# tenpy/cyten

Hardware: AMD Instinct MI355X
Metric: block-sparse tdot+SVD GFLOP/s (fp64) (higher is better)
Workload: dtype f64

## Files before the change

### cyten_amd/csrc/jacobi_engine.hip

```cpp
#include "jacobi_engine.h"

#include <algorithm>
#include <cmath>
#include <cstdlib>

namespace cyb {
constexpr double kPredictQuad = 16.0;
namespace {

typedef double d4 __attribute__((ext_vector_type(4)));
typedef double d2 __attribute__((ext_vector_type(2)));
#define GLOBAL_AS __attribute__((address_space(1)))
typedef const GLOBAL_AS d2* gc2;
typedef const GLOBAL_AS d2* gcp2;
typedef GLOBAL_AS double* gp;

constexpr int GS = JP + 2;
constexpr int QS = JP + 16;
constexpr int GK = 64;
constexpr int XS = GK + 2;
constexpr int NT = 256;
constexpr int NPAIR = JP / 2;
static_assert(JP == 32, "the wave tiling below assumes 32 x 32 pair problems");

// ... 818 lines not shown
                if (ab > 1e-300) {
                    jacobi_rot_bf(Hr[p * CS + p], Hr[q * CS + q], ab, c, sn, thr2);
                    pr = gr / ab;
                    pi = gi / ab;
                }
                rot[lane * 4 + 0] = c;
                rot[lane * 4 + 1] = sn;
                rot[lane * 4 + 2] = pr;
                rot[lane * 4 + 3] = pi;
            }
            __builtin_amdgcn_fence(__ATOMIC_RELEASE, "wavefront");
            __builtin_amdgcn_wave_barrier();
            for (int e = lane; e < (CJ / 2) * CJ; e += 64) {
                const int k = e / CJ, col = e % CJ;
                int p, q;
                pair_of(r, k, p, q);
                const double c = rot[k * 4], sn = rot[k * 4 + 1], fr = rot[k * 4 + 2], fi = rot[k * 4 + 3];
                const double pr_ = Hr[p * CS + col], pi_ = Hi[p * CS + col], qr_ = Hr[q * CS + col], qi_ = Hi[q * CS + col];
                const double tr = fr * qr_ - fi * qi_, ti = fr * qi_ + fi * qr_;
                Hr[p * CS + col] = c * pr_ - sn * tr;
                Hi[p * CS + col] = c * pi_ - sn * ti;
                Hr[q * CS + col] = sn * pr_ + c * tr;
                Hi[q * CS + col] = sn * pi_ + c * ti;
            }
            __builtin_amdgcn_fence(__ATOMIC_RELEASE, "wavefront");
            __builtin_amdgcn_wave_barrier();
            for (int e = lane; e < (CJ / 2) * CJ * 2; e += 64) {
                const int which = e / ((CJ / 2) * CJ), f = e % ((CJ / 2) * CJ);
                const int k = f / CJ, row = f % CJ;
                int p, q;
                pair_of(r, k, p, q);
                double* Xr = which ? Ur : Hr;
                double* Xi = which ? Ui : Hi;
                const double c = rot[k * 4], sn = rot[k * 4 + 1], fr = rot[k * 4 + 2], fi = -rot[k * 4 + 3];
                const double pr_ = Xr[row * CS + p], pi_ = Xi[row * CS + p], qr_ = Xr[row * CS + q], qi_ = Xi[row * CS + q];
                const double tr = fr * qr_ - fi * qi_, ti = fr * qi_ + fi * qr_;
                Xr[row * CS + p] = c * pr_ - sn * tr;
                Xi[row * CS + p] = c * pi_ - sn * ti;
                Xr[row * CS + q] = sn * pr_ + c * tr;
                Xi[row * CS + q] = sn * pi_ + c * ti;
            }
            __builtin_amdgcn_fence(__ATOMIC_RELEASE, "wavefront");
            __builtin_amdgcn_wave_barrier();
        }
    for (int e = lane; e < CJ * CJ; e += 64) {
        const int a = e / CJ, b = e % CJ;
        const double x = Ur[a * CS + b], y = Ui[a * CS + b];
        Vout[(2 * a) * VS + 2 * b] = x;
        Vout[(2 * a) * VS + 2 * b + 1] = -y;
        Vout[(2 * a + 1) * VS + 2 * b] = y;
        Vout[(2 * a + 1) * VS + 2 * b + 1] = x;
    }
    if (lane < CJ) {
        const double lam = Hr[lane * CS + lane];
        Gdiag[(2 * lane) * GS + 2 * lane] = lam;
        Gdiag[(2 * lane + 1) * GS + 2 * lane + 1] = lam;
    }
}

struct SScratch {
    double* gpart;
    unsigned int* ticket;
    unsigned int* ready;
    unsigned int* err;
    const int2* wgmap;
    const int2* wgent;
    unsigned long long* stamps;
    int stamp_round;
    int n_sweeps, n_mats;
    unsigned int* arrive;
    int* nsw;
    unsigned int* readyJ;
    int defer_j;
    int cross_every, cross_min_nb;
};
constexpr int SW_MAX_ENT = 64;

constexpr int SW_UN = 8;
constexpr int SW_PRE = 6;
constexpr int SWEEP_XREG = (4 * JP * GS > JP * GS + 2 * JP * VS) ? 4 * JP * GS : JP * GS + 2 * JP * VS;
constexpr int SWEEP_LDS_DOUBLES = JP * GS + SWEEP_XREG + 2 * JP * QS + 8;
constexpr size_t SWEEP_LDS_BYTES = 88 * 1024;
static_assert((size_t)SWEEP_LDS_DOUBLES * 8 + 1024 <= SWEEP_LDS_BYTES, "LDS request of the sweep kernel");
constexpr int SWEEP_WG_PER_CU = 1;

typedef unsigned int u32x2 __attribute__((ext_vector_type(2)));
union Q8 {
    u32x2 u;
    double d;
};

template <int SLEEP = 1>
__device__ __forceinline__ bool spin_until(const unsigned int* word, unsigned int target, unsigned int* err)
{
    const unsigned long long t0 = wall_clock64();
    unsigned int it = 0;
    while (__hip_atomic_load(word, __ATOMIC_RELAXED, __HIP_MEMORY_SCOPE_AGENT) < target) {
        __builtin_amdgcn_s_sleep(SLEEP);
        if ((++it & 63u) == 0u) {
            if (__hip_atomic_load(err, __ATOMIC_RELAXED, __HIP_MEMORY_SCOPE_AGENT) != 0u) return false;
            if (wall_clock64() - t0 > 100000000ull) {
                __hip_atomic_store(err, 1u, __ATOMIC_RELAXED, __HIP_MEMORY_SCOPE_AGENT);
                return false;
            }
        }
    }
    return true;
}

__device__ __forceinline__ void sweep_update_j(const __amdgpu_buffer_rsrc_t rsJ, const double* Qm, int P, int Q, int nvp, int j_begin,
                                               int nJ, int wave, int lane)
{
    const int un = lane & 15, ukq = lane >> 4;
    const double* ap0 = Qm + (lane >> 4) * QS + (lane & 15);
    const double* ap1 = ap0 + 16;
    double a0[JP / 4], a1[JP / 4];
#pragma unroll
    for (int kk = 0; kk < JP / 4; ++kk) {
        a0[kk] = ap0[kk * 4 * QS];
        a1[kk] = ap1[kk * 4 * QS];
    }
    auto off_of = [&](int c, int k) { return (unsigned int)(((int64_t)xrow(k, P, Q) * nvp + (j_begin + c) * 64 + wave * 16 + un) * 8); };
    auto load = [&](double (&x)[JP / 4], int c) {
#pragma unroll
        for (int kk = 0; kk < JP / 4; ++kk) {
            Q8 q;
            q.u = __builtin_amdgcn_raw_buffer_load_b64(rsJ, off_of(c, 4 * kk + ukq), 0, 16);
            x[kk] = q.d;
        }
    };
    double xb[JP / 4], xn[JP / 4];
    if (nJ > 0) load(xb, 0);
    for (int c = 0; c < nJ; ++c) {
        if (c + 1 < nJ) load(xn, c + 1);
        d4 acc[2] = {d4{0.0, 0.0, 0.0, 0.0}, d4{0.0, 0.0, 0.0, 0.0}};
#pragma unroll
        for (int kk = 0; kk < JP / 4; ++kk) {
            acc[0] = __builtin_amdgcn_mfma_f64_16x16x4f64(a0[kk], xb[kk], acc[0], 0, 0, 0);
            acc[1] = __builtin_amdgcn_mfma_f64_16x16x4f64(a1[kk], xb[kk], acc[1], 0, 0, 0);
        }
#pragma unroll
        for (int i = 0; i < 2; ++i)
#pragma unroll
            for (int q = 0; q < 4; ++q) {
                Q8 v;
                v.d = acc[i][q];
                __builtin_amdgcn_raw_buffer_store_b64(v.u, rsJ, off_of(c, i * 16 + (lane >> 4) + 4 * q), 0, 16);
            }
#pragma unroll
        for (int kk = 0; kk < JP / 4; ++kk) xb[kk] = xn[kk];
    }
}

template <bool CPLX>
__global__ void __launch_bounds__(NT, 1)
jacobi_sweep_kernel(const RPair* __restrict__ pairs, int max_inner, unsigned long long* __restrict__ offmax_bits, SScratch sc)
{
    extern __shared__ __attribute__((aligned(16))) double rsm[];
    double* Gs = rsm;
    double* G2 = Gs + JP * GS;
    double* Va = G2 + JP * GS;
    double* Vb = Va + JP * VS;
    double* Xc = G2;
    double* Qs0 = G2 + SWEEP_XREG;
    double* Qs1 = Qs0 + JP * QS;
    double* red = Qs1 + JP * QS;
    int* ibase = reinterpret_cast<int*>(red + 8);
    int* perm = ibase;
    int* zrow = ibase + JP;
    int* zout = ibase + 2 * JP;
    int* flags = ibase + 3 * JP;
    int* edone = flags + 4;

    const int tid = threadIdx.x;
    const int lane = tid & 63, wave = tid >> 6;
    const int2 went = sc.wgent ? sc.wgent[blockIdx.x] : make_int2((int)blockIdx.x, (int)blockIdx.x + 1);
    int max_rounds = 0;
    for (int e = went.x; e < went.y; ++e) max_rounds = max(max_rounds, pairs[sc.wgmap[e].x].nb - 1);
    const int n_sw = sc.n_sweeps;
    const bool one_entry = went.y - went.x == 1;
    int pendP = -1, pendQ = -1, pend_ground = 0;
    if (n_sw > 1) {
        if (tid < SW_MAX_ENT) edone[tid] = 0;
        __syncthreads();
    }
    for (int sw = 0; sw < n_sw; ++sw) {
    for (int round = 0; round < max_rounds; ++round)
    for (int ent = went.x; ent < went.y; ++ent) {
    const int2 wm = sc.wgmap[ent];
    const int pi = wm.x, part = wm.y;
    const RPair mt = pairs[pi];
    if (round >= mt.nb - 1) continue;
    if (n_sw > 1 && edone[ent - went.x]) continue;
    const int ground = sw * (mt.nb - 1) + round;
    const int G = mt.pad[0];
    unsigned int* ready = sc.ready + mt.pad[1];
    unsigned int* readyJ = sc.readyJ + mt.pad[1];
    unsigned int* ticket = sc.ticket + pi;
    double* Qs = (ground & 1) ? Qs1 : Qs0;
    const unsigned int pbytes = JP * JP * 8;
    const __amdgpu_buffer_rsrc_t rsW = __builtin_amdgcn_make_buffer_rsrc(mt.W, 0, (int)((size_t)mt.nvp * mt.lenp * 8), 0x00020000);
    const __amdgpu_buffer_rsrc_t rsJ =
        __builtin_amdgcn_make_buffer_rsrc(mt.J ? mt.J : mt.W, 0, mt.J ? (int)((size_t)mt.nvp * mt.nvp * 8) : 0, 0x00020000);
    const int cw = mt.lenp / 64, cj = mt.J ? mt.nvp / 64 : 0;
    const int w_begin = (int)((int64_t)part * cw / G), w_end = (int)((int64_t)(part + 1) * cw / G);
    const int j_begin = (int)((int64_t)part * cj / G), j_end = (int)((int64_t)(part + 1) * cj / G);
    const int nW = w_end - w_begin, nJ = j_end - j_begin;
    const bool defer = sc.defer_j && one_entry && G > 1 && nJ > 0 && round < mt.nb - 2;
    const int ct = defer ? nW : nW + nJ;
    const int pre_limit = (sc.defer_j && G > 1) ? min(ct, nW) : ct;
    const int un = lane & 15, ukq = lane >> 4;
#define SWEEP_STAMP(k)                                                                                            \
    do {                                                                                                          \
        if (sc.stamps && tid == 0 && round == sc.stamp_round) sc.stamps[(size_t)blockIdx.x * 8 + (k)] = wall_clock64(); \
    } while (0)

    {
        int P, Q;
        circle_pair(mt.nb, round, mt.slot, P, Q);
        if (P > Q) {
            const int t = P;
            P = Q;
            Q = t;
        }
        SWEEP_STAMP(0);
        __syncthreads();
        if (ground > 0) {
            if (tid == 0) {
                bool ok = spin_until(ready + (size_t)P * G + part, (unsigned int)ground, sc.err);
                ok = ok && spin_until(ready + (size_t)Q * G + part, (unsigned int)ground, sc.err);
                flags[1] = ok ? 1 : 0;
            }
            __syncthreads();
            if (!flags[1]) return;
        }
        SWEEP_STAMP(1);
        auto chunk_off = [&](int c, int k, bool& in_w) -> unsigned int {
            in_w = c < nW;
            const int ld = in_w ? mt.lenp : mt.nvp;
            const int cc = in_w ? w_begin + c : j_begin + (c - nW);
            return (unsigned int)(((int64_t)xrow(k, P, Q) * ld + cc * 64 + wave * 16 + un) * 8);
        };
        auto chunk_load = [&](int c, int k) -> double {
            bool in_w;
            const unsigned int off = chunk_off(c, k, in_w);
            Q8 q;
            q.u = in_w ? __builtin_amdgcn_raw_buffer_load_b64(rsW, off, 0, 16) : __builtin_amdgcn_raw_buffer_load_b64(rsJ, off, 0, 16);
            return q.d;
        };
        double xpre[SW_PRE][JP / 4];
        {
            const int ld = mt.lenp;
            d4 acc00 = d4{0.0, 0.0, 0.0, 0.0}, acc01 = acc00, acc11 = acc00;
            const int r = lane & 15, g2 = 2 * (lane >> 4);
            const unsigned int o0 = (unsigned int)(((int64_t)xrow(r, P, Q) * ld + g2) * 8);
            const unsigned int o1 = (unsigned int)(((int64_t)xrow(r + 16, P, Q) * ld + g2) * 8);
            const int c_begin = 8 * w_begin, c_end = 8 * w_end;
            constexpr int UN = SW_UN;
            d2 x0[UN], x1[UN], n0[UN], n1[UN];
            auto load = [&](d2 (&a0)[UN], d2 (&a1)[UN], int c0) {
#pragma unroll
                for (int u = 0; u < UN; ++u) {
                    const int c = min(c0 + 4 * u, c_end - 1);
                    Q16 qa, qb;
                    qa.u = __builtin_amdgcn_raw_buffer_load_b128(rsW, o0 + (unsigned int)c * 64u, 0, 16);
                    qb.u = __builtin_amdgcn_raw_buffer_load_b128(rsW, o1 + (unsigned int)c * 64u, 0, 16);
                    a0[u] = qa.d;
                    a1[u] = qb.d;
                }
            };
            if (c_begin + wave < c_end) load(x0, x1, c_begin + wave);
#pragma unroll
            for (int c = 0; c < SW_PRE; ++c) {
                if (c < pre_limit) {
#pragma unroll
                    for (int kk = 0; kk < JP / 4; ++kk) xpre[c][kk] = chunk_load(c, 4 * kk + ukq);
                }
            }
            for (int c0 = c_begin + wave; c0 < c_end; c0 += 4 * UN) {
                const bool more = c0 + 4 * UN < c_end;
                if (more) load(n0, n1, c0 + 4 * UN);
#pragma unroll
                for (int u = 0; u < UN; ++u) {
                    if (c0 + 4 * u < c_end) {
                        acc00 = __builtin_amdgcn_mfma_f64_16x16x4f64(x0[u].x, x0[u].x, acc00, 0, 0, 0);
                        acc01 = __builtin_amdgcn_mfma_f64_16x16x4f64(x0[u].x, x1[u].x, acc01, 0, 0, 0);
                        acc11 = __builtin_amdgcn_mfma_f64_16x16x4f64(x1[u].x, x1[u].x, acc11, 0, 0, 0);
                        acc00 = __builtin_amdgcn_mfma_f64_16x16x4f64(x0[u].y, x0[u].y, acc00, 0, 0, 0);
                        acc01 = __builtin_amdgcn_mfma_f64_16x16x4f64(x0[u].y, x1[u].y, acc01, 0, 0, 0);
                        acc11 = __builtin_amdgcn_mfma_f64_16x16x4f64(x1[u].y, x1[u].y, acc11, 0, 0, 0);
                    }
                }
                if (more) {
#pragma unroll
                    for (int u = 0; u < UN; ++u) {
                        x0[u] = n0[u];
                        x1[u] = n1[u];
                    }
                }
            }
            double* wpart = Xc + wave * (JP * GS);
#pragma unroll
            for (int q = 0; q < 4; ++q) {
                const int rr = (lane >> 4) + 4 * q, cc = lane & 15;
                wpart[rr * GS + cc] = acc00[q];
                wpart[rr * GS + 16 + cc] = acc01[q];
                wpart[(16 + cc) * GS + rr] = acc01[q];
                wpart[(16 + rr) * GS + 16 + cc] = acc11[q];
            }
        }
        __syncthreads();
        SWEEP_STAMP(2);
        {
            const int gi = tid >> 3, gj = 4 * (tid & 7);
            d2 lo = d2{0.0, 0.0}, hi = d2{0.0, 0.0};
#pragma unroll
            for (int w = 0; w < 4; ++w) {
                const double* src = Xc + w * (JP * GS) + gi * GS + gj;
                lo.x += src[0];
                lo.y += src[1];
                hi.x += src[2];
                hi.y += src[3];
            }
            if (G > 1) {
                const __amdgpu_buffer_rsrc_t rs_all = __builtin_amdgcn_make_buffer_rsrc(
                    sc.gpart + ((size_t)pi * 2 + (size_t)(ground & 1)) * RGMAX * (JP * JP), 0, (int)(pbytes * G), 0x00020000);
                Q16 a, b;
                a.d = lo;
                b.d = hi;
                const unsigned int off = (unsigned int)part * pbytes + (unsigned int)tid * 32u;
                __builtin_amdgcn_raw_buffer_store_b128(a.u, rs_all, off, 0, 16);
                __builtin_amdgcn_raw_buffer_store_b128(b.u, rs_all, off + 16u, 0, 16);
                asm volatile("s_waitcnt vmcnt(0)" ::: "memory");
                __syncthreads();
                if (tid == 0) __hip_atomic_fetch_add(ticket, 1u, __ATOMIC_RELAXED, __HIP_MEMORY_SCOPE_AGENT);
                if (pendP >= 0) {
                    if (tid == 0) {
                        bool ok = spin_until(readyJ + (size_t)pendP * G + part, (unsigned int)pend_ground, sc.err);
// ... 16 lines not shown
                if (!flags[1]) return;
                lo = d2{0.0, 0.0};
                hi = d2{0.0, 0.0};
                for (int g0 = 0; g0 < G; g0 += 4) {
                    Q16 pa[4], pb[4];
#pragma unroll
                    for (int g = 0; g < 4; ++g) {
                        if (g0 + g < G) {
                            pa[g].u = __builtin_amdgcn_raw_buffer_load_b128(rs_all, (unsigned int)(g0 + g) * pbytes + (unsigned int)tid * 32u, 0, 16);
                            pb[g].u = __builtin_amdgcn_raw_buffer_load_b128(rs_all, (unsigned int)(g0 + g) * pbytes + (unsigned int)tid * 32u + 16u, 0, 16);
                        }
                    }
#pragma unroll
                    for (int g = 0; g < 4; ++g) {
                        if (g0 + g < G) {
                            lo += pa[g].d;
                            hi += pb[g].d;
                        }
                    }
                }
            }
            double* dst = Gs + gi * GS + gj;
            dst[0] = lo.x;
            dst[1] = lo.y;
            dst[2] = hi.x;
            dst[3] = hi.y;
        }
        __syncthreads();
        SWEEP_STAMP(3);
        if (tid == 0) flags[0] = 0;
        __syncthreads();
        if (tid < JP) {
            double g = Gs[tid * GS + tid];
            if constexpr (CPLX) g = fmax(g, Gs[(tid ^ 1) * GS + (tid ^ 1)]);
            const int z = (g > 0.0 && g <= mt.thr2) ? 1 : 0;
            zrow[tid] = z;
            perm[tid] = tid;
            if (z) flags[0] = 1;
        }
        __syncthreads();
        const bool any_null = flags[0] != 0;
        if (any_null) {
            for (int e = tid; e < JP * JP; e += NT) {
                const int i = e / JP, j = e % JP;
                if (zrow[i] || zrow[j]) Gs[i * GS + j] = 0.0;
            }
            __syncthreads();
        }
        const double off = gram_offmax(Gs, red, tid);
        if (part == 0 && tid == 0) atomicMax(offmax_bits + (size_t)sw * sc.n_mats + mt.mat, (unsigned long long)__double_as_longlong(off));
        const bool skip = off <= mt.tol && !any_null;
        if (!skip) {
            double* Ga = Gs;
            double* Gb = G2;
            double* Vc = Va;
            double* Vn = Vb;
            bool pos_is_interleaved = false;
            const int cross_k = sc.cross_every > 0 ? sc.cross_every : max(4, (mt.nb + 2) / 4);
            const bool cross = sc.cross_every != 0 && !any_null && mt.nb >= sc.cross_min_nb && (round % cross_k) != 0;
            if constexpr (CPLX) {
                if (tid < 64) hermitian_pivot_solve(Gs, G2, Vb, Va, Gs, max_inner, tid, 0.25 * mt.tol * mt.tol, cross);
                __syncthreads();
            } else {
            auto cpos = [](int i) { return i < JB ? 2 * i : 2 * (i - JB) + 1; };
            pos_is_interleaved = cross;
            if (cross) {
                for (int e = tid; e < JP * JP; e += NT) {
                    const int i = e / JP, j = e % JP;
                    Gb[cpos(i) * GS + cpos(j)] = Ga[i * GS + j];
                }
                for (int e = tid; e < JP * VS; e += NT) Va[e] = (cpos(e / VS) == (e % VS)) ? 1.0 : 0.0;
                double* t = Ga;
                Ga = Gb;
                Gb = t;
            } else
                for (int e = tid; e < JP * VS; e += NT) Va[e] = ((e / VS) == (e % VS)) ? 1.0 : 0.0;
            __syncthreads();
            {
                const int pr = tid >> 4, pc = tid & 15;
                const int r0 = 2 * pr, c0 = 2 * pc;
                const int dr0 = cross ? r0 : ring_next(r0), dr1 = cross ? ((r0 + 3) & (JP - 1)) : ring_next(r0 + 1);
                const int dc0 = cross ? c0 : ring_next(c0), dc1 = cross ? ((c0 + 3) & (JP - 1)) : ring_next(c0 + 1);
                const int n_steps = cross ? JB : JP - 1;
                for (int sweep = 0; sweep < (off <= mt.tol ? 0 : max_inner); ++sweep) {
                    for (int r = 0; r < n_steps; ++r) {
                        const d2 g0 = *reinterpret_cast<const d2*>(Ga + r0 * GS + c0);
                        const d2 g1 = *reinterpret_cast<const d2*>(Ga + (r0 + 1) * GS + c0);
                        const d2 ac = *reinterpret_cast<const d2*>(Ga + c0 * GS + c0);
                        const double dc = Ga[(c0 + 1) * GS + c0 + 1];
                        const d2 v0 = *reinterpret_cast<const d2*>(Vc + r0 * VS + c0);
                        const d2 v1 = *reinterpret_cast<const d2*>(Vc + (r0 + 1) * VS + c0);
                        double c1, s1, c2, s2;
                        jacobi_rot_bf(ac.x, dc, ac.y, c2, s2, 0.25 * mt.tol * mt.tol);
                        const int rsrc = (lane & 48) | pr;
                        c1 = __shfl(c2, rsrc);
                        s1 = __shfl(s2, rsrc);
                        const double hik = c1 * g0.x - s1 * g1.x, hil = c1 * g0.y - s1 * g1.y;
                        const double hjk = s1 * g0.x + c1 * g1.x, hjl = s1 * g0.y + c1 * g1.y;
                        double nik = c2 * hik - s2 * hil, nil = s2 * hik + c2 * hil;
                        double njk = c2 * hjk - s2 * hjl, njl = s2 * hjk + c2 * hjl;
                        if (pr == pc) {
                            nil = 0.0;
                            njk = 0.0;
                        }
                        Gb[dr0 * GS + dc0] = nik;
                        Gb[dr0 * GS + dc1] = nil;
                        Gb[dr1 * GS + dc0] = njk;
                        Gb[dr1 * GS + dc1] = njl;
                        Vn[r0 * VS + dc0] = c2 * v0.x - s2 * v0.y;
                        Vn[r0 * VS + dc1] = s2 * v0.x + c2 * v0.y;
                        Vn[(r0 + 1) * VS + dc0] = c2 * v1.x - s2 * v1.y;
                        Vn[(r0 + 1) * VS + dc1] = s2 * v1.x + c2 * v1.y;
                        __syncthreads();
                        double* t = Ga;
                        Ga = Gb;
                        Gb = t;
                        t = Vc;
                        Vc = Vn;
                        Vn = t;
                    }
                    if (sweep + 1 < max_inner) {
                        const double off_in = gram_offmax(Ga, red, tid);
                        if (off_in <= 0.25 * mt.tol) break;
                    }
                }
            }
            }
            __syncthreads();
            SWEEP_STAMP(4);
            if (off > mt.tol && tid < 64) {
                const int li = lane & (JP - 1);
                const int li_idx = pos_is_interleaved ? ((li & 1) ? JB + (li >> 1) : (li >> 1)) : li;
                const double g = xrow(li_idx, P, Q) < mt.nv ? Ga[li * GS + li] : -1.0e300;
                const int glo = __double2loint(g), ghi = __double2hiint(g);
                int rk = 0;
#pragma unroll
                for (int j = 0; j < JP; ++j) {
                    const double gj = __hiloint2double(__builtin_amdgcn_readlane(ghi, j), __builtin_amdgcn_readlane(glo, j));
                    rk += (gj > g || (gj == g && j < li)) ? 1 : 0;
                }
                if (lane < JP) perm[rk] = lane;
            }
            __syncthreads();
            for (int e = tid; e < JP * JP; e += NT) {
                const int k = e / JP, m = e % JP;
                Qs[k * QS + m] = Vc[k * VS + perm[m]];
            }
            if (tid < JP) {
                const int pp = perm[tid];
                zout[tid] = zrow[pos_is_interleaved ? ((pp & 1) ? JB + (pp >> 1) : (pp >> 1)) : pp];
            }
            __syncthreads();
            SWEEP_STAMP(5);
            if (ct > nW) {
                if (tid == 0) {
                    bool ok = spin_until(readyJ + (size_t)P * G + part, (unsigned int)ground, sc.err);
                    ok = ok && spin_until(readyJ + (size_t)Q * G + part, (unsigned int)ground, sc.err);
                    flags[1] = ok ? 1 : 0;
                }
                __syncthreads();
                if (!flags[1]) return;
#pragma unroll
                for (int c = 0; c < SW_PRE; ++c) {
                    if (c >= pre_limit && c < ct) {
#pragma unroll
                        for (int kk = 0; kk < JP / 4; ++kk) xpre[c][kk] = chunk_load(c, 4 * kk + ukq);
                    }
                }
            }
            if (ct > 0) {
                const double* ap0 = Qs + (lane >> 4) * QS + (lane & 15);
                const double* ap1 = ap0 + 16;
                double a0[JP / 4], a1[JP / 4];
#pragma unroll
                for (int kk = 0; kk < JP / 4; ++kk) {
                    a0[kk] = ap0[kk * 4 * QS];
                    a1[kk] = ap1[kk * 4 * QS];
                }
                int zr[2][4];
#pragma unroll
                for (int i = 0; i < 2; ++i)
#pragma unroll
                    for (int q = 0; q < 4; ++q) zr[i][q] = zout[i * 16 + (lane >> 4) + 4 * q];
                auto apply = [&](int c, const double (&xb)[JP / 4]) {
                    d4 acc[2] = {d4{0.0, 0.0, 0.0, 0.0}, d4{0.0, 0.0, 0.0, 0.0}};
#pragma unroll
                    for (int kk = 0; kk < JP / 4; ++kk) {
                        acc[0] = __builtin_amdgcn_mfma_f64_16x16x4f64(a0[kk], xb[kk], acc[0], 0, 0, 0);
                        acc[1] = __builtin_amdgcn_mfma_f64_16x16x4f64(a1[kk], xb[kk], acc[1], 0, 0, 0);
                    }
                    const bool zero_null = c < nW;
#pragma unroll
                    for (int i = 0; i < 2; ++i)
#pragma unroll
                        for (int q = 0; q < 4; ++q) {
                            const int row = i * 16 + (lane >> 4) + 4 * q;
                            bool in_w;
                            const unsigned int o = chunk_off(c, row, in_w);
                            Q8 v;
                            v.d = (zero_null && zr[i][q]) ? 0.0 : acc[i][q];
                            if (in_w) __builtin_amdgcn_raw_buffer_store_b64(v.u, rsW, o, 0, 16);
                            else __builtin_amdgcn_raw_buffer_store_b64(v.u, rsJ, o, 0, 16);
                        }
                };
#pragma unroll
                for (int c = 0; c < SW_PRE; ++c)
                    if (c < ct) apply(c, xpre[c]);
                if (ct > SW_PRE) {
                    double xb[JP / 4], xn[JP / 4];
#pragma unroll
                    for (int kk = 0; kk < JP / 4; ++kk) xb[kk] = chunk_load(SW_PRE, 4 * kk + ukq);
                    for (int c = SW_PRE; c < ct; ++c) {
                        if (c + 1 < ct) {
#pragma unroll
                            for (int kk = 0; kk < JP / 4; ++kk) xn[kk] = chunk_load(c + 1, 4 * kk + ukq);
                        }
                        apply(c, xb);
#pragma unroll
                        for (int kk = 0; kk < JP / 4; ++kk) xb[kk] = xn[kk];
                    }
                }
            }
        }
        if (defer && !skip) {
            pendP = P;
            pendQ = Q;
            pend_ground = ground;
        }
        asm volatile("s_waitcnt vmcnt(0)" ::: "memory");
        __syncthreads();
        if (tid == 0) {
            if (skip && nJ > 0) {
                (void)spin_until(readyJ + (size_t)P * G + part, (unsigned int)ground, sc.err);
                (void)spin_until(readyJ + (size_t)Q * G + part, (unsigned int)ground, sc.err);
            }
            __hip_atomic_store(ready + (size_t)P * G + part, (unsigned int)(ground + 1), __ATOMIC_RELAXED, __HIP_MEMORY_SCOPE_AGENT);
            __hip_atomic_store(ready + (size_t)Q * G + part, (unsigned int)(ground + 1), __ATOMIC_RELAXED, __HIP_MEMORY_SCOPE_AGENT);
            if (!(defer && !skip)) {
                __hip_atomic_store(readyJ + (size_t)P * G + part, (unsigned int)(ground + 1), __ATOMIC_RELAXED, __HIP_MEMORY_SCOPE_AGENT);
                __hip_atomic_store(readyJ + (size_t)Q * G + part, (unsigned int)(ground + 1), __ATOMIC_RELAXED, __HIP_MEMORY_SCOPE_AGENT);
            }
            if (n_sw > 1 && round == mt.nb - 2) __hip_atomic_fetch_add(sc.arrive + mt.mat, 1u, __ATOMIC_RELAXED, __HIP_MEMORY_SCOPE_AGENT);
        }
        SWEEP_STAMP(6);
    }
    }
    if (n_sw == 1) break;
    __syncthreads();
    if (tid == 0) {
        int all = 1, ok = 1;
        for (int ent = went.x; ent < went.y && ok; ++ent) {
            if (edone[ent - went.x]) continue;
            const int2 wm = sc.wgmap[ent];
            const RPair mt = pairs[wm.x];
            const unsigned int entries = (unsigned int)(mt.nb / 2) * (unsigned int)mt.pad[0];
            if (!spin_until<32>(sc.arrive + mt.mat, entries * (unsigned int)(sw + 1), sc.err)) {
                ok = 0;
                break;
            }
            const double off = __longlong_as_double((long long)__hip_atomic_load(offmax_bits + (size_t)sw * sc.n_mats + mt.mat, __ATOMIC_RELAXED, __HIP_MEMORY_SCOPE_AGENT));
            const double prev = sw ? __longlong_as_double((long long)__hip_atomic_load(offmax_bits + (size_t)(sw - 1) * sc.n_mats + mt.mat,
                                                                                      __ATOMIC_RELAXED, __HIP_MEMORY_SCOPE_AGENT))
                                   : 1e300;
            const bool stagnated = sw + 1 >= 6 && off <= 64.0 * mt.tol && off >= 0.5 * prev;
            const bool predicted = off <= 0.1 * sqrt(mt.tol) && prev < 1.0 && off <= prev * sqrt(prev) && off <= kPredictQuad * prev * prev;
            if (off <= mt.tol || stagnated || predicted) {
                edone[ent - went.x] = 1;
                if (mt.slot == 0 && wm.y == 0) sc.nsw[mt.mat] = sw + 1;
            } else all = 0;
        }
        flags[1] = ok;
        flags[2] = all;
    }
    __syncthreads();
    if (!flags[1] || flags[2]) return;
    }
#undef SWEEP_STAMP
}

}

int jacobi_orthogonalise(cyb_ctx_t ctx, const std::vector<JMat>& h_mats, int max_sweeps,
                         std::vector<int32_t>& sweeps_out, bool cplx)
{
    const int n = (int)h_mats.size();
    sweeps_out.assign((size_t)n, 0);
    if (n == 0) return CYB_OK;
    hipStream_t st = ctx->stream;

    std::vector<int> active;
    for (int i = 0; i < n; ++i) {
        if (h_mats[(size_t)i].nv <= 1) sweeps_out[(size_t)i] = 0;
        else active.push_back(i);
    }
    static const bool one_launch_ok = getenv("CYB_JACOBI_PERSWEEP") == nullptr && getenv("CYB_JACOBI_TRACE") == nullptr &&
                                      getenv("CYB_JACOBI_STAMPS") == nullptr && getenv("CYB_JACOBI_NOPREDICT") == nullptr;
    static const bool one_launch_all = getenv("CYB_JACOBI_ONELAUNCH") != nullptr;
    int nb_max_all = 0;
    for (int i = 0; i < n; ++i) nb_max_all = std::max(nb_max_all, h_mats[(size_t)i].nb);
    const int n_sw_dev = (one_launch_ok && (one_launch_all || nb_max_all <= 16)) ? max_sweeps : 1;
    const size_t w_off = (size_t)n * (size_t)n_sw_dev;
    const size_t b_off = (sizeof(unsigned long long) * w_off + 2 * sizeof(unsigned int) * (size_t)n + 15) / 16 * 16;
    std::vector<unsigned long long> h_off(b_off / 8 + 2);
    bool one_launch_done = false;
    std::vector<int> cached_order, cached_G;
    uint64_t cached_at = 0;
    void* cached_img = nullptr;
    size_t cached_map_off = 0;
    std::vector<double> prev_off((size_t)n, 1e300);
    int status = CYB_OK;
    for (int sweep = 1; sweep <= max_sweeps && !active.empty(); ++sweep) {
        std::vector<int> order = active;
        std::stable_sort(order.begin(), order.end(),
                         [&](int a, int b) { return h_mats[(size_t)a].nb > h_mats[(size_t)b].nb; });
        std::vector<JWork> wl;
        int max_nb = 0;
        for (int m : order) {
            const int nb = h_mats[(size_t)m].nb;
            max_nb = std::max(max_nb, nb);
            for (int k = 0; k < nb / 2; ++k) wl.push_back(JWork{m, k});
        }
        const JMat* d_mats = nullptr;
        void* d_wl = nullptr;
        static const bool legacy = getenv("CYB_JACOBI_LEGACY") != nullptr;
        static const int fused_max = getenv("CYB_JACOBI_FUSED_MAX") ? atoi(getenv("CYB_JACOBI_FUSED_MAX")) : 64;
        static const int inner_env = getenv("CYB_JACOBI_INNER") ? atoi(getenv("CYB_JACOBI_INNER")) : 0;
        const int max_inner = inner_env > 0 ? inner_env : (max_nb <= 8 ? 3 : 1);
        constexpr int kGmax = RGMAX;
        const size_t np = wl.size();
        const size_t b_cnt = (sizeof(unsigned int) * np * (size_t)std::max(max_nb - 1, 1) + 15) / 16 * 16;
        const size_t b_gpart = sizeof(double) * np * kGmax * JP * JP, b_q = sizeof(double) * np * JP * JP;
        const size_t b_z = sizeof(int32_t) * np * JP, b_f = (sizeof(int32_t) * np + 15) / 16 * 16, b_c = (sizeof(unsigned int) * np + 15) / 16 * 16;
        size_t n_ready = 0;
        for (int m : order) n_ready += (size_t)h_mats[(size_t)m].nb * RGMAX;
        const size_t b_ready = (sizeof(unsigned int) * (2 * n_ready + np) + 15) / 16 * 16;
        void* wsp = nullptr;
        status = ctx->workspace(b_off + 16 + b_cnt + b_ready + 2 * b_gpart + 2 * (b_q + b_z + b_f) + b_c + 1024, &wsp, 2);
        if (status != CYB_OK) break;
        char* bp = static_cast<char*>(wsp);
        RScratch rs;
        unsigned long long* d_off = reinterpret_cast<unsigned long long*>(bp);
        rs.err = reinterpret_cast<unsigned int*>(bp + b_off);
        rs.cnt = reinterpret_cast<unsigned int*>(bp + b_off + 16);
        unsigned int* d_ready = reinterpret_cast<unsigned int*>(bp + b_off + 16 + b_cnt);
        bp += b_off + 16 + b_cnt + b_ready;
        rs.gpart = reinterpret_cast<double*>(bp);
        bp += 2 * b_gpart;
        rs.np = (int)np;
        rs.stamps = nullptr;
        JScratch sc;
        sc.gpart = rs.gpart;
        for (int h = 0; h < 2; ++h) {
            sc.qout[h] = reinterpret_cast<double*>(bp);
            bp += b_q;
        }
        for (int h = 0; h < 2; ++h) {
            sc.zout[h] = reinterpret_cast<int32_t*>(bp);
            bp += b_z;
        }
        for (int h = 0; h < 2; ++h) {
            sc.flag[h] = reinterpret_cast<int32_t*>(bp);
            bp += b_f;
        }
        sc.cnt = reinterpret_cast<unsigned int*>(bp);
        if (hipMemsetAsync(wsp, 0, b_off + 16 + b_cnt + b_ready, st) != hipSuccess) {
            status = CYB_ERR_HIP;
            break;
        }
        std::vector<RPair> rp(np);
        for (size_t k = 0; k < np; ++k) {
            const JMat& jm = h_mats[(size_t)wl[k].mat];
            RPair& q = rp[k];
            q.W = jm.W;
            q.J = jm.J;
            q.tol = jm.tol;
            q.thr2 = jm.thr2;
            q.nvp = jm.nvp;
            q.lenp = jm.lenp;
            q.nb = jm.nb;
            q.nv = jm.nv;
            q.mat = wl[k].mat;
            q.slot = wl[k].slot;
            q.pad[0] = q.pad[1] = 0;
        }
        void* d_rp = nullptr;
        static const bool want_stamps = getenv("CYB_JACOBI_STAMPS") != nullptr;
        static unsigned long long* d_stamps = nullptr;
        if (want_stamps) {
            if (!d_stamps && hipMalloc(reinterpret_cast<void**>(&d_stamps), sizeof(unsigned long long) * 8 * 2048) != hipSuccess) d_stamps = nullptr;
            rs.stamps = d_stamps;
        }
        static bool attr_set = false;
        if (!attr_set) {
            if (hipFuncSetAttribute(reinterpret_cast<const void*>(jacobi_round_kernel), hipFuncAttributeMaxDynamicSharedMemorySize,
                                    (int)ROUND_LDS_BYTES) != hipSuccess) {
                set_error("jacobi: cannot reserve %zu bytes of LDS for the round kernel", ROUND_LDS_BYTES);
                status = CYB_ERR_HIP;
                break;
            }
            attr_set = true;
        }
        bool any_j = false;
        for (int m : order) any_j = any_j || h_mats[(size_t)m].J != nullptr;
        static const bool defer_j = getenv("CYB_JACOBI_NODEFER") == nullptr;
        static const int g_env = getenv("CYB_JACOBI_G") ? atoi(getenv("CYB_JACOBI_G")) : 0;
        static const int u_max = getenv("CYB_JACOBI_UMAX") ? atoi(getenv("CYB_JACOBI_UMAX")) : 16;
        static const bool no_sweep = getenv("CYB_JACOBI_NOSWEEP") != nullptr;
        bool did_sweep = false;
        bool big_ok = true;
        for (int m : order)
            big_ok = big_ok && (size_t)h_mats[(size_t)m].nvp * (size_t)std::max(h_mats[(size_t)m].lenp, h_mats[(size_t)m].nvp) * 8 < ((size_t)1 << 31);
        const size_t sweep_slots = (size_t)SWEEP_WG_PER_CU * (size_t)ctx->n_cu;
        static const bool no_share = getenv("CYB_JACOBI_NOSHARE") != nullptr;
        if (!legacy && !no_sweep && big_ok && (np <= sweep_slots || !no_share)) {
            std::vector<int> Gm((size_t)n, 1);
            auto chain = [&](int m) {
                const JMat& jm = h_mats[(size_t)m];
                const double per_round = 8.0 + 22.0 * (double)(jm.lenp + ((jm.J || jm.rec_j) ? jm.nvp : 0)) / 2240.0 / (double)Gm[(size_t)m]
                                         + (Gm[(size_t)m] > 1 ? 4.0 : 0.0);
                return per_round * (double)(jm.nb - 1);
            };
            size_t used = np;
            while (true) {
                int best = -1;
                double worst = 0.0;
                for (int m : order) {
                    const JMat& jm = h_mats[(size_t)m];
                    const int cw_ = jm.lenp / 64;
                    if (Gm[(size_t)m] >= RGMAX || Gm[(size_t)m] >= cw_ || used + (size_t)jm.nb / 2 > sweep_slots) continue;
                    const double c = chain(m);
                    if (c > worst) {
                        worst = c;
                        best = m;
                    }
                }
                if (best < 0) break;
                ++Gm[(size_t)best];
                used += (size_t)h_mats[(size_t)best].nb / 2;
            }
            if (g_env > 0)
                for (int m : order) Gm[(size_t)m] = std::max(1, std::min({g_env, RGMAX, h_mats[(size_t)m].lenp / 64}));
            size_t total = 0;
            for (int m : order) total += (size_t)h_mats[(size_t)m].nb / 2 * (size_t)Gm[(size_t)m];
            if (total <= sweep_slots || (!no_share && total == np)) {
                std::vector<int> flag_base((size_t)n, 0);
                int fb = (int)np;
                for (int m : order) {
                    flag_base[(size_t)m] = fb;
                    fb += h_mats[(size_t)m].nb * Gm[(size_t)m];
                }
                std::vector<int2> wgmap;
                for (size_t k = 0; k < np; ++k) {
                    rp[k].pad[0] = Gm[(size_t)wl[k].mat];
                    rp[k].pad[1] = flag_base[(size_t)wl[k].mat];
                    for (int g = 0; g < Gm[(size_t)wl[k].mat]; ++g) wgmap.push_back(make_int2((int)k, g));
                }
                std::vector<int2> wgent;
                if (wgmap.size() > sweep_slots) {
                    std::vector<size_t> ent_before;
                    size_t acc = 0;
                    for (int m : order) {
                        ent_before.push_back(acc);
                        acc += (size_t)h_mats[(size_t)m].nb / 2;
                    }
                    ent_before.push_back(acc);
                    size_t best_i = 0, best_m = 0;
                    double best_cost = 1e300;
                    for (size_t i = 0; i <= order.size(); ++i) {
                        const size_t D = ent_before[i], S = acc - D;
                        if (D > sweep_slots || (S > 0 && D >= sweep_slots)) break;
                        const size_t m = S ? (S + (sweep_slots - D) - 1) / (sweep_slots - D) : 1;
                        const double own = (double)(h_mats[(size_t)order[0]].nb - 1);
                        const double shared = i < order.size() ? (double)m * (double)(h_mats[(size_t)order[i]].nb - 1) : 0.0;
                        const double cost = std::max(own, shared);
                        if (cost < best_cost) {
                            best_cost = cost;
                            best_i = i;
                            best_m = m;
                        }
                    }
                    const size_t D = ent_before[best_i];
                    for (size_t e = 0; e < D; ++e) wgent.push_back(make_int2((int)e, (int)e + 1));
                    for (size_t e = D; e < wgmap.size(); e += best_m)
                        wgent.push_back(make_int2((int)e, (int)std::min(e + best_m, wgmap.size())));
                }
                const size_t n_wg = wgent.empty() ? wgmap.size() : wgent.size();
                std::vector<int> g_now;
                for (int m : order) g_now.push_back(Gm[(size_t)m]);
                const size_t map_off = (sizeof(RPair) * np + 255) / 256 * 256;
                const size_t ent_off = (map_off + sizeof(int2) * wgmap.size() + 255) / 256 * 256;
                if (!(cached_img && order == cached_order && g_now == cached_G && ctx->n_uploads - cached_at < (uint64_t)cyb_ctx_s::kSlots / 2 - 1)) {
                    std::vector<char> img(ent_off + sizeof(int2) * wgent.size());
                    memcpy(img.data(), rp.data(), sizeof(RPair) * np);
                    memcpy(img.data() + map_off, wgmap.data(), sizeof(int2) * wgmap.size());
                    if (!wgent.empty()) memcpy(img.data() + ent_off, wgent.data(), sizeof(int2) * wgent.size());
                    status = ctx->upload(img.data(), img.size(), &cached_img);
                    if (status != CYB_OK) break;
                    cached_order = order;
                    cached_G = g_now;
                    cached_at = ctx->n_uploads;
                    cached_map_off = map_off;
                }
                void* d_rp2 = cached_img;
                void* d_map = static_cast<char*>(cached_img) + cached_map_off;
                static bool attr2_set = false;
                if (!attr2_set) {
                    if (hipFuncSetAttribute(reinterpret_cast<const void*>(jacobi_sweep_kernel<false>), hipFuncAttributeMaxDynamicSharedMemorySize,
                                            (int)SWEEP_LDS_BYTES) != hipSuccess ||
                        hipFuncSetAttribute(reinterpret_cast<const void*>(jacobi_sweep_kernel<true>), hipFuncAttributeMaxDynamicSharedMemorySize,
                                            (int)SWEEP_LDS_BYTES) != hipSuccess) {
                        set_error("jacobi: cannot reserve %zu bytes of LDS for the sweep kernel", SWEEP_LDS_BYTES);
                        status = CYB_ERR_HIP;
                        break;
                    }
                    attr2_set = true;
                }
                SScratch ss;
                ss.gpart = rs.gpart;
                ss.ticket = d_ready;
                ss.ready = d_ready;
                ss.readyJ = d_ready + n_ready;
                static const bool no_defer_j = getenv("CYB_JACOBI_NODEFERJ") != nullptr;
                ss.defer_j = no_defer_j ? 0 : 1;
                static const int cross_env = getenv("CYB_JACOBI_CROSS") ? atoi(getenv("CYB_JACOBI_CROSS")) : -1;
                static const bool cross_small = getenv("CYB_JACOBI_CROSS_SMALL") != nullptr;
                ss.cross_every = (max_inner == 1 || cross_small) ? cross_env : 0;
                static const int cross_min_nb = getenv("CYB_JACOBI_CROSS_MINNB") ? atoi(getenv("CYB_JACOBI_CROSS_MINNB")) : 0;
                ss.cross_min_nb = cross_min_nb;
                ss.err = rs.err;
                ss.wgmap = static_cast<const int2*>(d_map);
                ss.wgent = wgent.empty() ? nullptr : reinterpret_cast<const int2*>(static_cast<char*>(cached_img) + ent_off);
                ss.stamps = wgent.empty() ? rs.stamps : nullptr;
                ss.stamp_round = std::min(3, max_nb - 2);
                size_t max_ent = 1;
                for (const int2& we : wgent) max_ent = std::max(max_ent, (size_t)(we.y - we.x));
                const bool one_launch = n_sw_dev > 1 && sweep == 1 && max_ent <= (size_t)SW_MAX_ENT;
                ss.n_sweeps = one_launch ? n_sw_dev : 1;
                ss.n_mats = n;
                ss.arrive = reinterpret_cast<unsigned int*>(d_off + w_off);
                ss.nsw = reinterpret_cast<int*>(ss.arrive + n);
                one_launch_done = one_launch;
                if (cplx)
                    hipLaunchKernelGGL(jacobi_sweep_kernel<true>, dim3((unsigned)n_wg), dim3(NT), SWEEP_LDS_BYTES, st,
                                       static_cast<const RPair*>(d_rp2), max_inner, d_off, ss);
                else
                    hipLaunchKernelGGL(jacobi_sweep_kernel<false>, dim3((unsigned)n_wg), dim3(NT), SWEEP_LDS_BYTES, st,
                                       static_cast<const RPair*>(d_rp2), max_inner, d_off, ss);
                if (ss.stamps && wgmap.size() <= 2048) {
                    std::vector<unsigned long long> hs(8 * wgmap.size());
                    if (hipMemcpyAsync(hs.data(), rs.stamps, sizeof(unsigned long long) * hs.size(), hipMemcpyDeviceToHost, st) == hipSuccess &&
                        hipStreamSynchronize(st) == hipSuccess) {
                        double acc[6] = {0, 0, 0, 0, 0, 0};
                        int cntw = 0;
                        const int mbig = order.front();
                        for (size_t b = 0; b < wgmap.size(); ++b) {
                            if (wl[(size_t)wgmap[b].x].mat != mbig) continue;
                            for (int k = 0; k < 6; ++k) acc[k] += (double)(hs[8 * b + k + 1] - hs[8 * b + k]) * 0.01;
                            ++cntw;
                        }
                        if (cntw)
                            fprintf(stderr, "[jacobi sweep stamps] sweep %d round %d, largest matrix (G=%d, %d workgroups of %zu): wait %.2f load+gram %.2f "
                                            "exch %.2f defl+eig %.2f sort %.2f upd+publish %.2f us\n",
                                    sweep, ss.stamp_round, Gm[(size_t)mbig], cntw, wgmap.size(), acc[0] / cntw, acc[1] / cntw,
                                    acc[2] / cntw, acc[3] / cntw, acc[4] / cntw, acc[5] / cntw);
                    }
                }
                did_sweep = true;
            }
        }
        if (!did_sweep && cplx) {
            set_error("block-Jacobi on embedded complex rows needs the persistent sweep kernel (list too large for one launch)");
            status = CYB_ERR_UNSUPPORTED;
            break;
        }
        if (!did_sweep) {
        cached_img = nullptr;
        {
            void* d_mats_v = nullptr;
            status = ctx->upload(h_mats.data(), sizeof(JMat) * (size_t)n, &d_mats_v);
            if (status == CYB_OK) status = ctx->upload(wl.data(), sizeof(JWork) * wl.size(), &d_wl);
            if (status == CYB_OK) status = ctx->upload(rp.data(), sizeof(RPair) * np, &d_rp);
            if (status != CYB_OK) break;
            d_mats = static_cast<const JMat*>(d_mats_v);
            if (hipMemsetAsync(sc.cnt, 0, b_c, st) != hipSuccess) {
                status = CYB_ERR_HIP;
                break;
            }
        }
        int pend_round = -1;
        size_t pend_cnt = 0;
        auto flush_pending = [&]() {
            if (pend_round < 0) return;
            const int U = (int)std::min<size_t>(16, std::max<size_t>(1, (size_t)(3 * ctx->n_cu) / pend_cnt));
            hipLaunchKernelGGL(jacobi_update_kernel, dim3((unsigned)(pend_cnt * U)), dim3(NT), 0, st, d_mats,
                               static_cast<const JWork*>(d_wl), pend_round, U, sc, pend_round & 1, 0, 1);
            pend_round = -1;
        };
        for (int r = 0; r < max_nb - 1; ++r) {
            size_t cnt = 0;
            for (int m : order) {
                if (h_mats[(size_t)m].nb - 1 > r) cnt += (size_t)h_mats[(size_t)m].nb / 2;
                else break;
            }
            if (cnt == 0) break;
            const bool fused = !legacy && cnt <= (size_t)fused_max && cnt <= (size_t)ctx->n_cu;
            if (fused) {
                flush_pending();
                int G = (int)std::min<size_t>(kGmax, (size_t)ctx->n_cu / cnt);
                if (g_env > 0 && (size_t)g_env * cnt <= (size_t)ctx->n_cu) G = std::min(g_env, kGmax);
                G = std::max(G, 1);
                hipLaunchKernelGGL(jacobi_round_kernel, dim3((unsigned)(cnt * G)), dim3(NT), ROUND_LDS_BYTES, st,
                                   static_cast<const RPair*>(d_rp), r, G, max_inner, d_off, rs);
                if (rs.stamps && r == max_nb / 2 && cnt * (size_t)G <= 2048) {
                    std::vector<unsigned long long> hs(8 * cnt * G);
                    if (hipMemcpyAsync(hs.data(), rs.stamps, sizeof(unsigned long long) * hs.size(), hipMemcpyDeviceToHost, st) == hipSuccess &&
                        hipStreamSynchronize(st) == hipSuccess) {
                        double acc[6] = {0, 0, 0, 0, 0, 0}, tot = 0, mx = 0;
                        for (size_t b = 0; b < cnt * G; ++b) {
                            for (int k = 0; k < 6; ++k) acc[k] += (double)(hs[8 * b + k + 1] - hs[8 * b + k]) * 0.01;
                            const double t = (double)(hs[8 * b + 6] - hs[8 * b]) * 0.01;
                            tot += t;
                            mx = std::max(mx, t);
                        }
                        const double nb_ = (double)(cnt * G);
                        fprintf(stderr, "[jacobi stamps] sweep %d round %d: %zu pairs x G=%d | gram %.2f exch %.2f defl %.2f eig %.2f sort %.2f upd %.2f | wg mean %.2f max %.2f us\n",
                                sweep, r, cnt, G, acc[0] / nb_, acc[1] / nb_, acc[2] / nb_, acc[3] / nb_, acc[4] / nb_, acc[5] / nb_, tot / nb_, mx);
                    }
                }
                continue;
            }
            const int slots = 2 * ctx->n_cu;
            int G = g_env > 0 ? g_env : ((size_t)2 * cnt <= (size_t)slots ? 2 : 1);
            G = std::min(G, kGmax);
            const int U = (int)std::min<size_t>((size_t)u_max, std::max<size_t>(1, (size_t)(3 * ctx->n_cu) / cnt));
            const int buf = r & 1;
            const int n_gram = (int)(cnt * G);
            int UJ = 1;
            size_t n_jwg = 0;
            if (pend_round >= 0) {
                const long long free_slots = (long long)slots - (long long)n_gram;
                UJ = (int)std::max<long long>(1, std::min<long long>(8, free_slots / (long long)pend_cnt));
                n_jwg = pend_cnt * (size_t)UJ;
            }
            hipLaunchKernelGGL(jacobi_gram_kernel, dim3((unsigned)(n_gram + n_jwg)), dim3(NT), 0, st, d_mats,
                               static_cast<const JWork*>(d_wl), r, G, max_inner, d_off, sc, buf, n_gram, pend_round, UJ);
            const bool defer = defer_j && any_j;
            hipLaunchKernelGGL(jacobi_update_kernel, dim3((unsigned)(cnt * U)), dim3(NT), 0, st, d_mats,
                               static_cast<const JWork*>(d_wl), r, U, sc, buf, 1, defer ? 0 : 1);
            pend_round = defer ? r : -1;
            pend_cnt = cnt;
        }
        flush_pending();
        }
        if (hipGetLastError() != hipSuccess) {
            set_error("jacobi round kernels: launch failed");
            status = CYB_ERR_HIP;
            break;
        }
        unsigned int h_err = 0;
        if (ctx->d2h(h_off.data(), d_off, b_off + 16) != CYB_OK) {
            set_error("jacobi: reading the convergence flags failed: %s", hipGetErrorString(hipGetLastError()));
            status = CYB_ERR_HIP;
            break;
        }
        memcpy(&h_err, reinterpret_cast<const char*>(h_off.data()) + b_off, sizeof(unsigned int));
        if (h_err) {
            set_error("jacobi round kernel: a workgroup waited more than a second for the Gram partials of its pair "
                      "(partner workgroup not resident?)");
            status = CYB_ERR_HIP;
            break;
        }
        std::vector<int> still;
        if (one_launch_done) {
            const int* h_nsw = reinterpret_cast<const int*>(reinterpret_cast<const unsigned int*>(h_off.data() + w_off) + n);
            for (int m : active) {
                if (h_nsw[m] > 0) sweeps_out[(size_t)m] = h_nsw[m];
                else still.push_back(m);
            }
            active.swap(still);
            break;
        }
        static const bool trace = getenv("CYB_JACOBI_TRACE") != nullptr;
        for (int m : active) {
            double off;
            memcpy(&off, &h_off[(size_t)m], sizeof(double));
            if (trace)
                fprintf(stderr, "[jacobi] sweep %2d mat %3d (nv=%d len=%d) off=%.3e tol=%.3e\n", sweep, m,
                        h_mats[(size_t)m].nv, h_mats[(size_t)m].len, off, h_mats[(size_t)m].tol);
            const double tol = h_mats[(size_t)m].tol;
            const bool stagnated = sweep >= 6 && off <= 64.0 * tol && off >= 0.5 * prev_off[(size_t)m];
            static const bool no_predict = getenv("CYB_JACOBI_NOPREDICT") != nullptr;
            const double prev = prev_off[(size_t)m];
            const bool predicted = !no_predict && off <= 0.1 * std::sqrt(tol) && prev < 1.0 && off <= prev * std::sqrt(prev) &&
                                   off <= kPredictQuad * prev * prev;
            if (off <= tol || stagnated || predicted) sweeps_out[(size_t)m] = sweep;
            else still.push_back(m);
            prev_off[(size_t)m] = off;
        }
        active.swap(still);
    }
    if (status != CYB_OK) return status;
    if (!active.empty()) {
        for (int m : active) sweeps_out[(size_t)m] = -1;
        set_error("block-Jacobi did not converge within %d sweeps for %zu matrices", max_sweeps, active.size());
        return CYB_ERR_NOCONV;
    }
    return CYB_OK;
}

}
```

Before: 5447.

## Move per-sweep convergence verdict into round zero and enable one-launch for all sizes

Replaces the end-of-sweep block-wide convergence barrier with a per-entry verdict check at the start of the next sweep. Each workgroup now waits only on the arrival counter of the matrix it is about to work on, and retires converged entries individually instead of waiting for all its entries. The single persistent multi-sweep launch is also enabled regardless of the largest block count (previously capped at nb<=16), and it is now allowed when stamps are on. Stamp instrumentation for the verdict waits is added. The risks are correctness of the new sync protocol and longer spin waits on large matrices that now run in one launch.

```diff
diff --git a/cyten_amd/csrc/jacobi_engine.hip b/cyten_amd/csrc/jacobi_engine.hip
--- a/cyten_amd/csrc/jacobi_engine.hip
+++ b/cyten_amd/csrc/jacobi_engine.hip
@@ -994,6 +994,17 @@
     }
 }
 
+__device__ __forceinline__ bool sweep_stops(const unsigned long long* offmax_bits, int n_mats, int mat, int s, double tol)
+{
+    const double off = __longlong_as_double((long long)__hip_atomic_load(offmax_bits + (size_t)s * n_mats + mat, __ATOMIC_RELAXED, __HIP_MEMORY_SCOPE_AGENT));
+    const double prev = s ? __longlong_as_double((long long)__hip_atomic_load(offmax_bits + (size_t)(s - 1) * n_mats + mat,
+                                                                             __ATOMIC_RELAXED, __HIP_MEMORY_SCOPE_AGENT))
+                          : 1e300;
+    const bool stagnated = s + 1 >= 6 && off <= 64.0 * tol && off >= 0.5 * prev;
+    const bool predicted = off <= 0.1 * sqrt(tol) && prev < 1.0 && off <= prev * sqrt(prev) && off <= kPredictQuad * prev * prev;
+    return off <= tol || stagnated || predicted;
+}
+
 template <bool CPLX>
 __global__ void __launch_bounds__(NT, 1)
 jacobi_sweep_kernel(const RPair* __restrict__ pairs, int max_inner, unsigned long long* __restrict__ offmax_bits, SScratch sc)
@@ -1026,6 +1037,8 @@
         if (tid < SW_MAX_ENT) edone[tid] = 0;
         __syncthreads();
     }
+    int n_live = went.y - went.x;
+    unsigned long long vwait = 0;
     for (int sw = 0; sw < n_sw; ++sw) {
     for (int round = 0; round < max_rounds; ++round)
     for (int ent = went.x; ent < went.y; ++ent) {
@@ -1348,6 +1361,34 @@
             }
             __syncthreads();
             SWEEP_STAMP(5);
+        }
+        if (n_sw > 1 && sw > 0 && round == 0) {
+            if (tid == 0) {
+                const unsigned long long t0 = sc.stamps ? wall_clock64() : 0ull;
+                const unsigned int entries = (unsigned int)(mt.nb / 2) * (unsigned int)G;
+                int v = 2;
+                if (spin_until(sc.arrive + mt.mat, entries * (unsigned int)sw, sc.err)) {
+                    v = sweep_stops(offmax_bits, sc.n_mats, mt.mat, sw - 1, mt.tol) ? 1 : 0;
+                    if (v) {
+                        edone[ent - went.x] = 1;
+                        if (mt.slot == 0 && part == 0) sc.nsw[mt.mat] = sw;
+                    }
+                }
+                flags[3] = v;
+                if (sc.stamps) {
+                    vwait += wall_clock64() - t0;
+                    sc.stamps[(size_t)blockIdx.x * 8 + 7] = vwait;
+                }
+            }
+            __syncthreads();
+            const int v = flags[3];
+            if (v == 2) return;
+            if (v == 1) {
+                if (--n_live == 0) return;
+                continue;
+            }
+        }
+        if (!skip) {
             if (ct > nW) {
                 if (tid == 0) {
                     bool ok = spin_until(readyJ + (size_t)P * G + part, (unsigned int)ground, sc.err);
@@ -1441,35 +1482,20 @@
         SWEEP_STAMP(6);
     }
     }
+    if (sw + 1 < n_sw) continue;
     if (n_sw == 1) break;
     __syncthreads();
     if (tid == 0) {
-        int all = 1, ok = 1;
-        for (int ent = went.x; ent < went.y && ok; ++ent) {
+        for (int ent = went.x; ent < went.y; ++ent) {
             if (edone[ent - went.x]) continue;
             const int2 wm = sc.wgmap[ent];
             const RPair mt = pairs[wm.x];
+            if (mt.slot != 0 || wm.y != 0) continue;
             const unsigned int entries = (unsigned int)(mt.nb / 2) * (unsigned int)mt.pad[0];
-            if (!spin_until<32>(sc.arrive + mt.mat, entries * (unsigned int)(sw + 1), sc.err)) {
-                ok = 0;
-                break;
-            }
-            const double off = __longlong_as_double((long long)__hip_atomic_load(offmax_bits + (size_t)sw * sc.n_mats + mt.mat, __ATOMIC_RELAXED, __HIP_MEMORY_SCOPE_AGENT));
-            const double prev = sw ? __longlong_as_double((long long)__hip_atomic_load(offmax_bits + (size_t)(sw - 1) * sc.n_mats + mt.mat,
-                                                                                      __ATOMIC_RELAXED, __HIP_MEMORY_SCOPE_AGENT))
-                                   : 1e300;
-            const bool stagnated = sw + 1 >= 6 && off <= 64.0 * mt.tol && off >= 0.5 * prev;
-            const bool predicted = off <= 0.1 * sqrt(mt.tol) && prev < 1.0 && off <= prev * sqrt(prev) && off <= kPredictQuad * prev * prev;
-            if (off <= mt.tol || stagnated || predicted) {
-                edone[ent - went.x] = 1;
-                if (mt.slot == 0 && wm.y == 0) sc.nsw[mt.mat] = sw + 1;
-            } else all = 0;
-        }
-        flags[1] = ok;
-        flags[2] = all;
-    }
-    __syncthreads();
-    if (!flags[1] || flags[2]) return;
+            if (!spin_until<32>(sc.arrive + mt.mat, entries * (unsigned int)(sw + 1), sc.err)) break;
+            if (sweep_stops(offmax_bits, sc.n_mats, mt.mat, sw, mt.tol)) sc.nsw[mt.mat] = sw + 1;
+        }
+    }
     }
 #undef SWEEP_STAMP
 }
@@ -1490,11 +1516,9 @@
         else active.push_back(i);
     }
     static const bool one_launch_ok = getenv("CYB_JACOBI_PERSWEEP") == nullptr && getenv("CYB_JACOBI_TRACE") == nullptr &&
-                                      getenv("CYB_JACOBI_STAMPS") == nullptr && getenv("CYB_JACOBI_NOPREDICT") == nullptr;
+                                      getenv("CYB_JACOBI_NOPREDICT") == nullptr;
     static const bool one_launch_all = getenv("CYB_JACOBI_ONELAUNCH") != nullptr;
-    int nb_max_all = 0;
-    for (int i = 0; i < n; ++i) nb_max_all = std::max(nb_max_all, h_mats[(size_t)i].nb);
-    const int n_sw_dev = (one_launch_ok && (one_launch_all || nb_max_all <= 16)) ? max_sweeps : 1;
+    const int n_sw_dev = (one_launch_ok && (one_launch_all || true)) ? max_sweeps : 1;
     const size_t w_off = (size_t)n * (size_t)n_sw_dev;
     const size_t b_off = (sizeof(unsigned long long) * w_off + 2 * sizeof(unsigned int) * (size_t)n + 15) / 16 * 16;
     std::vector<unsigned long long> h_off(b_off / 8 + 2);
@@ -1736,6 +1760,7 @@
                 ss.arrive = reinterpret_cast<unsigned int*>(d_off + w_off);
                 ss.nsw = reinterpret_cast<int*>(ss.arrive + n);
                 one_launch_done = one_launch;
+                if (ss.stamps && one_launch && hipMemsetAsync(ss.stamps, 0, sizeof(unsigned long long) * 8 * 2048, st) != hipSuccess) ss.stamps = nullptr;
                 if (cplx)
                     hipLaunchKernelGGL(jacobi_sweep_kernel<true>, dim3((unsigned)n_wg), dim3(NT), SWEEP_LDS_BYTES, st,
                                        static_cast<const RPair*>(d_rp2), max_inner, d_off, ss);
@@ -1759,6 +1784,19 @@
                                             "exch %.2f defl+eig %.2f sort %.2f upd+publish %.2f us\n",
                                     sweep, ss.stamp_round, Gm[(size_t)mbig], cntw, wgmap.size(), acc[0] / cntw, acc[1] / cntw,
                                     acc[2] / cntw, acc[3] / cntw, acc[4] / cntw, acc[5] / cntw);
+                        if (one_launch && cntw) {
+                            double vs = 0.0, vm = 0.0;
+                            for (size_t b = 0; b < wgmap.size(); ++b) {
+                                if (wl[(size_t)wgmap[b].x].mat != mbig) continue;
+                                vs += (double)hs[8 * b + 7] * 0.01;
+                                vm = std::max(vm, (double)hs[8 * b + 7] * 0.01);
+                            }
+                            int nsw_big = 0;
+                            (void)ctx->d2h(&nsw_big, ss.nsw + mbig, sizeof(int));
+                            fprintf(stderr, "[jacobi sweep stamps] one launch, largest matrix: %d sweeps, verdict waits of a workgroup summed over the "
+                                            "launch: mean %.2f max %.2f us\n",
+                                    nsw_big, vs / cntw, vm);
+                        }
                     }
                 }
                 did_sweep = true;
```

New measurement: 5529 (median of 2 runs). No clear change (+1.5%).
